# AppleHolic/pytorch_sound

Measured on AMD Instinct MI355X. Metric: audio-sec/s STFT+mel+fwd/bwd, higher is better.
Workload: dtype bf16; 1 GPU; configs[1]: Conv1d separator (4 x ResBlock1, C=256, on 513-bin magnitude), 22.05 kHz, STFT 1024/256, 80 mel, batch 32 x 2 s per GPU, Adam, bf16 autocast; global_batch=32, parallelism=dp1, model_params=5520386

## Files before the change

### pytorch_sound_amd/csrc/psnd_conv_chain.hip

```cpp
#include "psnd_conv_pair.h"

#include <atomic>
extern std::atomic<long long> g_conv_pair_stats[4];
std::atomic<long long> g_conv_chain_stats[2];

namespace {
using namespace pairk;

constexpr int CHAIN_MAX = 4;
struct ChainPair {
    const bf16_t *W1, *W2;
    const float *bias1, *bias2;
    bf16_t *mid_out, *out_raw, *out_act;
    int off1, dstep1, off2, dstep2;
    float act1_slope, act2_slope;
    const bf16_t *M1, *M2;
    float m1_slope, m2_slope;
};
struct ChainParams {
    const bf16_t *A, *res;
    long long R;
    int Lp, L, HP;
    int n_pairs, lo, ts;
    ChainPair d[CHAIN_MAX];
    long long *trace;
};
#define CHAIN_STAMP(i_)                                                                  \
    do {                                                                                 \
        if (p.trace && (threadIdx.x & 63) == 0) p.trace[((size_t)blockIdx.x * 8 + (threadIdx.x >> 6)) * 16 + (i_)] = __builtin_amdgcn_s_memtime(); \
    } while (0)

template <int C, int MR, bool BWD>
__global__ __launch_bounds__(512, 1) void conv_chain_kernel(ChainParams p) {
    constexpr int NT = 512, RU = RU8;
#ifndef PSND_CHAIN_AR
#define PSND_CHAIN_AR 3
#endif
    constexpr int AR = PSND_CHAIN_AR;
    static_assert(RU % AR == 0, "static ring slots");
    constexpr int RS = C + 8, PCS = C / 8, KSTEPS = C / 16, UNITS = 3 * KSTEPS;
    constexpr int MROWS = 32 * MR, MB = MR, BR = MROWS + 2 * HMAXP;
    static_assert(C == 256, "eight waves = eight column blocks of 32");
    static_assert(UNITS % RU == 0 && RU % 3 == 0, "the B ring turns whole");
    extern __shared__ __attribute__((aligned(16))) bf16_t smem[];
    __shared__ unsigned char s_in[MROWS];
    __shared__ __attribute__((aligned(16))) float s_bias[BWD ? 1 : 2][BWD ? 4 : 2 * C];
    __shared__ unsigned s_flag[2];
#ifndef PSND_CHAIN_FLAGS
#define PSND_CHAIN_FLAGS 0
#endif
    constexpr bool FLAGS = PSND_CHAIN_FLAGS != 0;
#ifndef PSND_CHAIN_EPRIO
#define PSND_CHAIN_EPRIO 2
#endif
    if (threadIdx.x < 2) s_flag[threadIdx.x] = 0;
    auto wait_flag = [&](int g, unsigned need) __attribute__((always_inline)) {
        if (!FLAGS || need == 0) return;
        volatile unsigned *f = &s_flag[g];
        int spins = 0;
        while (*f < need) {
            __builtin_amdgcn_s_sleep(1);
            if (++spins > (1 << 24)) __builtin_trap();
        }
        __builtin_amdgcn_fence(__ATOMIC_ACQUIRE, "workgroup");
    };
    auto signal_flag = [&]() __attribute__((always_inline)) {
        if (!FLAGS) return;
        __builtin_amdgcn_fence(__ATOMIC_RELEASE, "workgroup");
        if ((threadIdx.x & 63) == 0) __hip_atomic_fetch_add(&s_flag[threadIdx.x >> 8], 1u, __ATOMIC_RELAXED, __HIP_MEMORY_SCOPE_WORKGROUP);
    };
    bf16_t *sXa = smem, *sM = smem + BR * RS, *sXr = smem + 2 * BR * RS;
    const int tid = threadIdx.x, wave = tid >> 6, lane = tid & 63, li = lane & 31, kg = lane >> 5;
    const int cb = wave * 32 + 4 * kg, eo = li * RS + cb;
    const long long g0 = (long long)blockIdx.x * p.ts - p.lo;
    const unsigned t_bytes = (unsigned)((size_t)p.R * C * sizeof(bf16_t)), w_bytes = (unsigned)(3u * C * C * sizeof(bf16_t));
    const __amdgpu_buffer_rsrc_t rA = make_uniform_rsrc(p.A, (int)t_bytes), rR = make_uniform_rsrc(p.res, (int)t_bytes);
    CHAIN_STAMP(0);

    constexpr int NAU = (BR * PCS + NT - 1) / NT, NRU = MROWS * PCS / NT;
    static_assert(NRU * NT == MROWS * PCS, "raw tile tiling");
    uint4 ra[NAU], rr[BWD ? 1 : NRU];
#pragma unroll
    for (int u = 0; u < NAU; ++u) {
        const int idx = tid + NT * u, row = idx / PCS, pc = idx % PCS;
        const long long r = g0 - HMAXP + row;
        ra[u] = ld16(rA, (idx < BR * PCS && r >= 0 && r < p.R) ? (unsigned)(((size_t)r * C + 8 * pc) * sizeof(bf16_t)) : OOB);
    }
    if constexpr (!BWD) {
#pragma unroll
        for (int u = 0; u < NRU; ++u) {
            const int idx = tid + NT * u, row = idx / PCS, pc = idx % PCS;
            const long long r = g0 + row;
            rr[u] = ld16(rR, (r >= 0 && r < p.R) ? (unsigned)(((size_t)r * C + 8 * pc) * sizeof(bf16_t)) : OOB);
        }
    }
    unsigned char *sBits = reinterpret_cast<unsigned char *>(smem + 2 * BR * RS);
    constexpr int NMU = MROWS * PCS / NT;
    uint4 mq[BWD ? NMU : 1];
    auto mask_fetch = [&](const bf16_t *M) __attribute__((always_inline)) {
        const __amdgpu_buffer_rsrc_t rM = make_uniform_rsrc(M, (int)t_bytes);
#pragma unroll
        for (int u = 0; u < NMU; ++u) {
            const int idx = tid + NT * u, row = idx / PCS, pc = idx % PCS;
            const long long r = g0 + row;
            mq[u] = ld16(rM, (r >= 0 && r < p.R) ? (unsigned)(((size_t)r * C + 8 * pc) * sizeof(bf16_t)) : OOB);
        }
    };
    auto mask_commit = [&](int buf) __attribute__((always_inline)) {
#pragma unroll
        for (int u = 0; u < NMU; ++u) {
            const unsigned *w = reinterpret_cast<const unsigned *>(&mq[u]);
            unsigned byte = 0;
#pragma unroll
            for (int e = 0; e < 4; ++e) {
                byte |= ((int)(w[e] << 16) > 0 ? 1u : 0u) << (2 * e);
                byte |= ((int)w[e] > 0xffff ? 1u : 0u) << (2 * e + 1);
            }
            sBits[buf * (MROWS * PCS) + tid + NT * u] = (unsigned char)byte;
        }
    };
    if constexpr (BWD) mask_fetch(p.d[0].M1);
    uint4 rb[RU];
    const unsigned fwave = (unsigned)wave * (unsigned)KSTEPS * 1024u + (unsigned)lane * 16u;
    constexpr unsigned FTAP = (unsigned)(C / 32) * (unsigned)KSTEPS * 1024u;
    auto fetch_b = [&](auto slotc, __amdgpu_buffer_rsrc_t rW, int it) __attribute__((always_inline)) {
        constexpr int slot = decltype(slotc)::value, tap = slot % 3, ksl = slot / 3;
        const int ks = (RU / 3) * it + ksl;
        rb[slot] = __builtin_bit_cast(uint4, __builtin_amdgcn_raw_buffer_load_b128(rW, (int)(ks < KSTEPS ? fwave : OOB),
                                                                                    (int)((unsigned)tap * FTAP + (unsigned)ks * 1024u), 0));
    };
    {
        const __amdgpu_buffer_rsrc_t rW = make_uniform_rsrc(p.d[0].W1, (int)w_bytes);
        static_for<0, RU>([&](auto uc) __attribute__((always_inline)) { fetch_b(uc, rW, 0); });
    }
    ChainPair d = p.d[0];
    if constexpr (!BWD) {
        const float *bp = tid < C ? d.bias1 : d.bias2;
        s_bias[0][tid] = bp ? bp[tid & (C - 1)] : 0.f;
    }
    if (tid < MROWS) {
        const long long r = g0 + tid;
        const int l = (int)(((r % p.Lp) + p.Lp) % p.Lp);
        s_in[tid] = (r >= 0 && r < p.R && l >= p.HP && l < p.HP + p.L) ? 1 : 0;
    }
#pragma unroll
    for (int u = 0; u < NAU; ++u) {
        const int idx = tid + NT * u;
        if (idx < BR * PCS) *reinterpret_cast<uint4 *>(sXa + (idx / PCS) * RS + 8 * (idx % PCS)) = ra[u];
    }
    if constexpr (!BWD) {
#pragma unroll
        for (int u = 0; u < NRU; ++u) {
            const int idx = tid + NT * u;
            *reinterpret_cast<uint4 *>(sXr + (idx / PCS) * RS + 8 * (idx % PCS)) = rr[u];
        }
    } else {
        mask_commit(0);
    }
    for (int idx = tid; idx < 2 * HMAXP * PCS; idx += NT) {
        const int row = idx / PCS < HMAXP ? idx / PCS : MROWS + idx / PCS;
        *reinterpret_cast<uint4 *>(sM + row * RS + 8 * (idx % PCS)) = make_uint4(0, 0, 0, 0);
    }
    __syncthreads();
    CHAIN_STAMP(1);
    float xres[MB][16];
#pragma unroll
    for (int m = 0; m < MB; ++m)
#pragma unroll
        for (int g = 0; g < 4; ++g) {
            const bf16_t *src = BWD ? sXa + HMAXP * RS : sXr;
            const uint2 w = *reinterpret_cast<const uint2 *>(src + eo + m * 32 * RS + 8 * g);
            xres[m][4 * g] = __builtin_bit_cast(float, w.x << 16), xres[m][4 * g + 1] = __builtin_bit_cast(float, w.x & 0xffff0000u);
            xres[m][4 * g + 2] = __builtin_bit_cast(float, w.y << 16), xres[m][4 * g + 3] = __builtin_bit_cast(float, w.y & 0xffff0000u);
        }

    f32x16 acc[MB];
    auto zero_acc = [&]() __attribute__((always_inline)) {
#pragma unroll
        for (int m = 0; m < MB; ++m)
#pragma unroll
            for (int i = 0; i < 16; ++i) acc[m][i] = 0.f;
    };
    auto run_conv = [&](const bf16_t *src, int off0, int dstep, __amdgpu_buffer_rsrc_t rW, __amdgpu_buffer_rsrc_t rWn, unsigned need) __attribute__((always_inline)) {
        wait_flag(0, need);
        const bf16_t *ab[3];
#pragma unroll
        for (int t = 0; t < 3; ++t) ab[t] = src + (li + HMAXP + off0 + t * dstep) * RS + 8 * kg;
        auto afrag = [&](auto uc, int it, bf16x8 (&x)[MB]) __attribute__((always_inline)) {
            constexpr int u = decltype(uc)::value, tap = u % 3, ksl = u / 3;
            const bf16_t *pa = ab[tap] + 16 * ((RU / 3) * it + ksl);
#pragma unroll
            for (int m = 0; m < MB; ++m) x[m] = *reinterpret_cast<const bf16x8 *>(pa + m * 32 * RS);
        };
        bf16x8 xr[AR][MB];
        auto turns = [&](int it0, int it1) __attribute__((always_inline)) {
            static_for<0, AR - 1>([&](auto uc) __attribute__((always_inline)) { afrag(uc, it0, xr[decltype(uc)::value]); });
#pragma unroll 1
            for (int it = it0; it < it1; ++it) {
                static_for<0, RU>([&](auto uc) __attribute__((always_inline)) {
                    constexpr int u = decltype(uc)::value;
                    afrag(std::integral_constant<int, u + AR - 1>{}, it, xr[(u + AR - 1) % AR]);
                    const bf16x8 b = __builtin_bit_cast(bf16x8, rb[u]);
#pragma unroll
                    for (int m = 0; m < MB; ++m) acc[m] = __builtin_amdgcn_mfma_f32_32x32x16_bf16(b, xr[u % AR][m], acc[m], 0, 0, 0);
                    fetch_b(uc, it + 1 < UNITS / RU ? rW : rWn, it + 1 < UNITS / RU ? it + 1 : 0);
                    __builtin_amdgcn_sched_group_barrier(0x100, MB, 0);
                    __builtin_amdgcn_sched_group_barrier(0x008, MB, 0);
                    __builtin_amdgcn_sched_group_barrier(0x020, 1, 0);
                    __builtin_amdgcn_sched_barrier(0);
                });
            }
        };
        if constexpr (FLAGS) {
            turns(0, UNITS / RU / 2);
            wait_flag(1, need);
            turns(UNITS / RU / 2, UNITS / RU);
        } else {
            turns(0, UNITS / RU);
        }
    };
    auto copy_out = [&](const bf16_t *src, int row_off, bf16_t *dst) __attribute__((always_inline)) {
        if (wave >= 4) return;
        const __amdgpu_buffer_rsrc_t rO = make_uniform_rsrc(dst, (int)t_bytes);
        for (int idx = tid; idx < p.ts * PCS; idx += NT / 2) {
            const int i = p.lo + idx / PCS, pc = idx % PCS;
            const long long r = g0 + i;
            const uint4 v = *reinterpret_cast<const uint4 *>(src + (row_off + i) * RS + 8 * pc);
            __builtin_amdgcn_raw_buffer_store_b128(__builtin_bit_cast(__attribute__((ext_vector_type(4))) unsigned, v), rO,
                                                   (int)(r < p.R ? (unsigned)(((size_t)r * C + 8 * pc) * 2) : OOB), 0, 0);
        }
    };

    unsigned rmask[MB];
#pragma unroll
    for (int m = 0; m < MB; ++m) rmask[m] = s_in[m * 32 + li] ? 0xffffffffu : 0u;
    bf16_t *prev_raw = nullptr, *prev_act = nullptr;
    auto st8 = [&](bf16_t *row0, int m, int g, unsigned w0, unsigned w1) __attribute__((always_inline)) {
        *reinterpret_cast<uint2 *>(row0 + eo + m * 32 * RS + 8 * g) = make_uint2(w0, w1);
    };
    auto bias4 = [&](int buf, int conv, float4 (&bb)[4]) __attribute__((always_inline)) {
#pragma unroll
        for (int g = 0; g < 4; ++g) bb[g] = *reinterpret_cast<const float4 *>(&s_bias[buf][conv * C + cb + 8 * g]);
    };
    auto mask32 = [&](int buf, int m) __attribute__((always_inline)) {
        return *reinterpret_cast<const unsigned *>(sBits + buf * (MROWS * PCS) + (m * 32 + li) * PCS + 4 * wave) >> (4 * kg);
    };
    auto masked = [&](float v, float slope, unsigned bits, int j) __attribute__((always_inline)) {
        const unsigned sel = (unsigned)(((int)(bits << (31 - j))) >> 31);
        return __builtin_bit_cast(float, (__builtin_bit_cast(unsigned, v) & sel) | (__builtin_bit_cast(unsigned, v * slope) & ~sel));
    };
#pragma unroll 1
    for (int pp = 0; pp < p.n_pairs; ++pp) {
        const ChainPair dn = p.d[pp + 1 < p.n_pairs ? pp + 1 : pp];
        float bn = 0.f;
        if constexpr (!BWD) {
            const float *bp = tid < C ? dn.bias1 : dn.bias2;
            bn = bp ? bp[tid & (C - 1)] : 0.f;
        }
        const float sl1 = d.act1_slope, sl2 = d.act2_slope, ms1 = d.m1_slope, ms2 = d.m2_slope;
        const __amdgpu_buffer_rsrc_t rW1 = make_uniform_rsrc(d.W1, (int)w_bytes), rW2 = make_uniform_rsrc(d.W2, (int)w_bytes);
        const __amdgpu_buffer_rsrc_t rWn = make_uniform_rsrc(dn.W1, pp + 1 < p.n_pairs ? (int)w_bytes : 0);
        if constexpr (BWD) mask_fetch(d.M2);
        zero_acc();
        run_conv(sXa, d.off1, d.dstep1, rW1, rW2, 8u * pp);
        if constexpr (FLAGS) __builtin_amdgcn_s_setprio(PSND_CHAIN_EPRIO);
        CHAIN_STAMP(2 + 4 * pp);
        if (pp > 0) {
            if (prev_raw) copy_out(BWD ? sXa : sXr, BWD ? HMAXP : 0, prev_raw);
            if (!BWD && prev_act) copy_out(sXa, HMAXP, prev_act);
        }
        if constexpr (BWD) {
#pragma unroll
            for (int m = 0; m < MB; ++m) {
                const unsigned bits = mask32(0, m);
#pragma unroll
                for (int g = 0; g < 4; ++g) {
                    float v[4];
#pragma unroll
                    for (int j = 0; j < 4; ++j) v[j] = masked(acc[m][4 * g + j], ms1, bits, 8 * g + j);
                    st8(sM + HMAXP * RS, m, g, pack_bf16(v[0], v[1]) & rmask[m], pack_bf16(v[2], v[3]) & rmask[m]);
                }
            }
            mask_commit(1);
        } else {
            float4 bb[4];
            bias4(pp & 1, 0, bb);
#pragma unroll
            for (int m = 0; m < MB; ++m)
#pragma unroll
                for (int g = 0; g < 4; ++g) {
                    const float v0 = acc[m][4 * g] + bb[g].x, v1 = acc[m][4 * g + 1] + bb[g].y;
                    const float v2 = acc[m][4 * g + 2] + bb[g].z, v3 = acc[m][4 * g + 3] + bb[g].w;
                    st8(sM + HMAXP * RS, m, g, pack_bf16(fmaxf(v0, v0 * sl1), fmaxf(v1, v1 * sl1)) & rmask[m],
                        pack_bf16(fmaxf(v2, v2 * sl1), fmaxf(v3, v3 * sl1)) & rmask[m]);
                }
            s_bias[(pp + 1) & 1][tid] = bn;
        }
        if (pp == 1) CHAIN_STAMP(14);
        if constexpr (FLAGS) {
            signal_flag();
            __builtin_amdgcn_s_setprio(0);
        } else {
            __syncthreads();
        }
        CHAIN_STAMP(3 + 4 * pp);
        if constexpr (BWD) mask_fetch(dn.M1);
        zero_acc();
        run_conv(sM, d.off2, d.dstep2, rW2, rWn, 8u * pp + 4u);
        if constexpr (FLAGS) __builtin_amdgcn_s_setprio(PSND_CHAIN_EPRIO);
        CHAIN_STAMP(4 + 4 * pp);
        if (d.mid_out) copy_out(sM, HMAXP, d.mid_out);
        if constexpr (BWD) {
#pragma unroll
            for (int m = 0; m < MB; ++m) {
                const unsigned bits = mask32(1, m);
#pragma unroll
                for (int g = 0; g < 4; ++g) {
                    unsigned w[2];
#pragma unroll
                    for (int h = 0; h < 2; ++h) {
                        const int q = 4 * g + 2 * h;
                        const float v0 = masked(acc[m][q], ms2, bits, 8 * g + 2 * h) + xres[m][q];
                        const float v1 = masked(acc[m][q + 1], ms2, bits, 8 * g + 2 * h + 1) + xres[m][q + 1];
                        w[h] = pack_bf16(v0, v1) & rmask[m];
                        xres[m][q] = __builtin_bit_cast(float, w[h] << 16), xres[m][q + 1] = __builtin_bit_cast(float, w[h] & 0xffff0000u);
                    }
                    st8(sXa + HMAXP * RS, m, g, w[0], w[1]);
                }
            }
            mask_commit(0);
        } else {
            float4 bb[4];
            bias4(pp & 1, 1, bb);
#pragma unroll
            for (int m = 0; m < MB; ++m)
#pragma unroll
                for (int g = 0; g < 4; ++g) {
                    const float bq[4] = {bb[g].x, bb[g].y, bb[g].z, bb[g].w};
                    unsigned w[2], wa[2];
#pragma unroll
                    for (int h = 0; h < 2; ++h) {
                        const int q = 4 * g + 2 * h;
                        const float v0 = acc[m][q] + bq[2 * h] + xres[m][q], v1 = acc[m][q + 1] + bq[2 * h + 1] + xres[m][q + 1];
                        w[h] = pack_bf16(v0, v1) & rmask[m];
                        xres[m][q] = __builtin_bit_cast(float, w[h] << 16), xres[m][q + 1] = __builtin_bit_cast(float, w[h] & 0xffff0000u);
                        wa[h] = pack_bf16(fmaxf(v0, v0 * sl2), fmaxf(v1, v1 * sl2)) & rmask[m];
                    }
                    st8(sXr, m, g, w[0], w[1]);
                    st8(sXa + HMAXP * RS, m, g, wa[0], wa[1]);
                }
        }
        if (pp == 1) CHAIN_STAMP(15);
        if constexpr (FLAGS) {
            signal_flag();
            __builtin_amdgcn_s_setprio(0);
        } else {
            __syncthreads();
        }
        CHAIN_STAMP(5 + 4 * pp);
        prev_raw = d.out_raw, prev_act = d.out_act;
        d = dn;
    }
    if constexpr (FLAGS) __syncthreads();
    if (prev_raw) copy_out(BWD ? sXa : sXr, BWD ? HMAXP : 0, prev_raw);
    if (!BWD && prev_act) copy_out(sXa, HMAXP, prev_act);
}

int chain_loss(const int *taps, int n_pairs) {
    int loss = 0;
    for (int i = 0; i < n_pairs; ++i) loss += reach3(taps[4 * i], taps[4 * i + 1]) + reach3(taps[4 * i + 2], taps[4 * i + 3]);
    return loss - reach3(taps[0], taps[1]);
}
}

extern "C" int psnd_conv1d_cl_chain_rows(int C, int k, int n_pairs, const int *taps) {
    if (k != 3 || C != 256 || n_pairs < 1 || n_pairs > CHAIN_MAX || !taps) return 0;
    for (int i = 0; i < 2 * n_pairs; ++i)
        if (reach3(taps[2 * i], taps[2 * i + 1]) > HMAXP) return 0;
    const int ts = 64 - 2 * chain_loss(taps, n_pairs);
    return ts >= 16 ? ts : 0;
}

extern "C" int psnd_conv1d_cl_chain_plan(int C, int k, int n_pairs, const int *taps, int64_t R, int *mr_out) {
    const int ts2 = psnd_conv1d_cl_chain_rows(C, k, n_pairs, taps);
    if (!ts2) return 0;
    const int ts1 = ts2 - 32;
    (void)R;
    int mr = 2;
    if (const char *e = PSND_ENV("PSND_CHAIN_MR")) {
        const int f = atoi(e);
        if (f == 2 || (f == 1 && ts1 >= 8)) mr = f;
    }
    if (mr_out) *mr_out = mr;
    return mr == 1 ? ts1 : ts2;
}

extern "C" int psnd_conv1d_cl_chain(const void *A, const void *res, const psnd_chain_pair *pairs, int n_pairs, int64_t N, int Lp, int L, int HP,
                                    int C, int k, void *stream) {
    if (!A || !res || !pairs) PSND_FAIL(PSND_E_ARG, "conv1d_cl_chain: null pointer");
    const bool bwd = n_pairs >= 1 && pairs[0].M1 != nullptr;
    if (N < 0 || Lp <= 0 || L <= 0 || HP < 0 || Lp < L + HP) PSND_FAIL(PSND_E_SHAPE, "conv1d_cl_chain: N=%lld Lp=%d L=%d HP=%d", (long long)N, Lp, L, HP);
    if (n_pairs < 1 || n_pairs > CHAIN_MAX) PSND_FAIL(PSND_E_UNSUPPORTED, "conv1d_cl_chain: %d pairs (1 ... %d)", n_pairs, CHAIN_MAX);
    int taps[4 * CHAIN_MAX];
    for (int i = 0; i < n_pairs; ++i) {
        taps[4 * i] = pairs[i].off1, taps[4 * i + 1] = pairs[i].dstep1, taps[4 * i + 2] = pairs[i].off2, taps[4 * i + 3] = pairs[i].dstep2;
        if (!pairs[i].W1 || !pairs[i].W2) PSND_FAIL(PSND_E_ARG, "conv1d_cl_chain: pair %d without weights", i);
        if (bwd != (pairs[i].M1 != nullptr) || bwd != (pairs[i].M2 != nullptr))
            PSND_FAIL(PSND_E_ARG, "conv1d_cl_chain: pair %d: masks on every conv of the chain (the input-gradient form) or on none", i);
        if (bwd && (res != A || pairs[i].act1_slope != 1.f || pairs[i].act2_slope != 1.f || pairs[i].out_act || pairs[i].bias1 || pairs[i].bias2))
            PSND_FAIL(PSND_E_UNSUPPORTED, "conv1d_cl_chain: pair %d: the masked (input-gradient) form has res == A, no activation, no bias, no out_act", i);
        if (!(pairs[i].act1_slope >= 0.f && pairs[i].act1_slope <= 1.f && pairs[i].act2_slope >= 0.f && pairs[i].act2_slope <= 1.f))
            PSND_FAIL(PSND_E_UNSUPPORTED, "conv1d_cl_chain: activation slopes %g, %g of pair %d outside [0, 1]", pairs[i].act1_slope, pairs[i].act2_slope, i);
    }
    int mr = 2;
    const int ts = psnd_conv1d_cl_chain_plan(C, k, n_pairs, taps, N * (int64_t)Lp, &mr);
    if (!ts) PSND_FAIL(PSND_E_UNSUPPORTED, "conv1d_cl_chain: C=%d k=%d, %d pairs: only k = 3, C = 256, reach <= %d, >= 16 rows left of 64", C, k, n_pairs, HMAXP);
    if (N == 0) return PSND_OK;
    if ((size_t)N * Lp * C * 2 >= ((size_t)1 << 31)) PSND_FAIL(PSND_E_SHAPE, "conv1d_cl_chain: operand larger than 2 GB");
    ChainParams p;
    p.A = static_cast<const bf16_t *>(A), p.res = static_cast<const bf16_t *>(res);
    p.R = N * (int64_t)Lp, p.Lp = Lp, p.L = L, p.HP = HP;
    p.n_pairs = n_pairs, p.ts = ts, p.lo = (32 * mr - ts) / 2;
    for (int i = 0; i < CHAIN_MAX; ++i) {
        const psnd_chain_pair &s = pairs[i < n_pairs ? i : n_pairs - 1];
        ChainPair &d = p.d[i];
        d.W1 = static_cast<const bf16_t *>(s.W1), d.W2 = static_cast<const bf16_t *>(s.W2), d.bias1 = s.bias1, d.bias2 = s.bias2;
        d.mid_out = static_cast<bf16_t *>(s.mid_out), d.out_raw = static_cast<bf16_t *>(s.out_raw), d.out_act = static_cast<bf16_t *>(s.out_act);
        d.off1 = s.off1, d.dstep1 = s.dstep1, d.off2 = s.off2, d.dstep2 = s.dstep2, d.act1_slope = s.act1_slope, d.act2_slope = s.act2_slope;
        d.M1 = static_cast<const bf16_t *>(s.M1), d.M2 = static_cast<const bf16_t *>(s.M2), d.m1_slope = s.m1_slope, d.m2_slope = s.m2_slope;
    }
    p.trace = nullptr;
#ifdef PSND_TRACE
    {
        const char *tp = PSND_ENV("PSND_PAIR_TRACE_PTR");
        p.trace = tp ? reinterpret_cast<long long *>(strtoull(tp, nullptr, 0)) : nullptr;
    }
#endif
    const int64_t tiles = (p.R + ts - 1) / ts;
    constexpr int RS = 256 + 8;
    const int mrows = 32 * mr;
    const size_t lds = bwd ? (size_t)2 * (mrows + 2 * HMAXP) * RS * 2 + 2 * 256 * 8 : (size_t)(2 * (mrows + 2 * HMAXP) + mrows) * RS * 2;
    hipStream_t st = static_cast<hipStream_t>(stream);
    auto launch = [&](auto kern) {
        hipFuncSetAttribute(reinterpret_cast<const void *>(kern), hipFuncAttributeMaxDynamicSharedMemorySize, 128 * 1024);
        hipLaunchKernelGGL(kern, dim3((unsigned)tiles), dim3(512), lds, st, p);
    };
    if (bwd && mr == 2) launch(conv_chain_kernel<256, 2, true>);
    else if (bwd) launch(conv_chain_kernel<256, 1, true>);
    else if (mr == 2) launch(conv_chain_kernel<256, 2, false>);
    else launch(conv_chain_kernel<256, 1, false>);
    PSND_CHECK_LAUNCH("conv1d_cl_chain");
    g_conv_chain_stats[0]++;
    g_conv_chain_stats[1] += n_pairs;
    return PSND_OK;
}

extern "C" void psnd_conv_chain_stats(long long *out2) {
    out2[0] = g_conv_chain_stats[0].load(), out2[1] = g_conv_chain_stats[1].load();
}
```

Before: 107,700 audio-s/s.

## Micro-optimize conv chain kernel: packed epilogues, fused acc zeroing, batched copy-out

Several micro-optimizations land in the fused conv chain kernel. The accumulator zeroing is folded into the first MFMA turn, and epilogue math uses packed f32x2 ops with bfe/bfi inline asm for the masked leaky-ReLU backward. Mask bit packing switches to packed u16 inline asm. The prologue is reordered so bias loads and halo zeroing are issued earlier, with sched barriers between weight prefetches. Copy-out precomputes offsets, batches LDS reads before the stores, and uses all 512 threads for the final store. Together these aim to cut VALU and scheduling overhead, at the cost of more complex code and inline asm whose correctness must hold across edge cases.

```diff
diff --git a/pytorch_sound_amd/csrc/psnd_conv_chain.hip b/pytorch_sound_amd/csrc/psnd_conv_chain.hip
--- a/pytorch_sound_amd/csrc/psnd_conv_chain.hip
+++ b/pytorch_sound_amd/csrc/psnd_conv_chain.hip
@@ -77,6 +77,12 @@
     const __amdgpu_buffer_rsrc_t rA = make_uniform_rsrc(p.A, (int)t_bytes), rR = make_uniform_rsrc(p.res, (int)t_bytes);
     CHAIN_STAMP(0);
 
+    ChainPair d = p.d[0];
+    float b0 = 0.f;
+    if constexpr (!BWD) {
+        const float *bp = tid < C ? d.bias1 : d.bias2;
+        b0 = bp ? bp[tid & (C - 1)] : 0.f;
+    }
     constexpr int NAU = (BR * PCS + NT - 1) / NT, NRU = MROWS * PCS / NT;
     static_assert(NRU * NT == MROWS * PCS, "raw tile tiling");
     uint4 ra[NAU], rr[BWD ? 1 : NRU];
@@ -110,13 +116,15 @@
 #pragma unroll
         for (int u = 0; u < NMU; ++u) {
             const unsigned *w = reinterpret_cast<const unsigned *>(&mq[u]);
-            unsigned byte = 0;
+            unsigned s = 0;
 #pragma unroll
             for (int e = 0; e < 4; ++e) {
-                byte |= ((int)(w[e] << 16) > 0 ? 1u : 0u) << (2 * e);
-                byte |= ((int)w[e] > 0xffff ? 1u : 0u) << (2 * e + 1);
+                unsigned x;
+                asm("v_pk_sub_u16 %0, %1, %2" : "=v"(x) : "v"(w[e]), "v"(0x00010001u));
+                asm("v_pk_add_u16 %0, %1, %2 clamp" : "=v"(x) : "v"(x), "v"(0x00800080u));
+                s |= (x >> (15 - 2 * e)) & (0x00010001u << (2 * e));
             }
-            sBits[buf * (MROWS * PCS) + tid + NT * u] = (unsigned char)byte;
+            sBits[buf * (MROWS * PCS) + tid + NT * u] = (unsigned char)~(s | (s >> 15));
         }
     };
     if constexpr (BWD) mask_fetch(p.d[0].M1);
@@ -131,18 +139,21 @@
     };
     {
         const __amdgpu_buffer_rsrc_t rW = make_uniform_rsrc(p.d[0].W1, (int)w_bytes);
-        static_for<0, RU>([&](auto uc) __attribute__((always_inline)) { fetch_b(uc, rW, 0); });
-    }
-    ChainPair d = p.d[0];
-    if constexpr (!BWD) {
-        const float *bp = tid < C ? d.bias1 : d.bias2;
-        s_bias[0][tid] = bp ? bp[tid & (C - 1)] : 0.f;
+        static_for<0, RU>([&](auto uc) __attribute__((always_inline)) {
+            fetch_b(uc, rW, 0);
+            __builtin_amdgcn_sched_barrier(0);
+        });
     }
     if (tid < MROWS) {
         const long long r = g0 + tid;
         const int l = (int)(((r % p.Lp) + p.Lp) % p.Lp);
         s_in[tid] = (r >= 0 && r < p.R && l >= p.HP && l < p.HP + p.L) ? 1 : 0;
     }
+    for (int idx = tid; idx < 2 * HMAXP * PCS; idx += NT) {
+        const int row = idx / PCS < HMAXP ? idx / PCS : MROWS + idx / PCS;
+        *reinterpret_cast<uint4 *>(sM + row * RS + 8 * (idx % PCS)) = make_uint4(0, 0, 0, 0);
+    }
+    if constexpr (!BWD) s_bias[0][tid] = b0;
 #pragma unroll
     for (int u = 0; u < NAU; ++u) {
         const int idx = tid + NT * u;
@@ -157,30 +168,20 @@
     } else {
         mask_commit(0);
     }
-    for (int idx = tid; idx < 2 * HMAXP * PCS; idx += NT) {
-        const int row = idx / PCS < HMAXP ? idx / PCS : MROWS + idx / PCS;
-        *reinterpret_cast<uint4 *>(sM + row * RS + 8 * (idx % PCS)) = make_uint4(0, 0, 0, 0);
-    }
     __syncthreads();
     CHAIN_STAMP(1);
-    float xres[MB][16];
+    f32x2_t xres[MB][8];
 #pragma unroll
     for (int m = 0; m < MB; ++m)
 #pragma unroll
         for (int g = 0; g < 4; ++g) {
             const bf16_t *src = BWD ? sXa + HMAXP * RS : sXr;
             const uint2 w = *reinterpret_cast<const uint2 *>(src + eo + m * 32 * RS + 8 * g);
-            xres[m][4 * g] = __builtin_bit_cast(float, w.x << 16), xres[m][4 * g + 1] = __builtin_bit_cast(float, w.x & 0xffff0000u);
-            xres[m][4 * g + 2] = __builtin_bit_cast(float, w.y << 16), xres[m][4 * g + 3] = __builtin_bit_cast(float, w.y & 0xffff0000u);
+            xres[m][2 * g] = f32x2_t{__builtin_bit_cast(float, w.x << 16), __builtin_bit_cast(float, w.x & 0xffff0000u)};
+            xres[m][2 * g + 1] = f32x2_t{__builtin_bit_cast(float, w.y << 16), __builtin_bit_cast(float, w.y & 0xffff0000u)};
         }
 
     f32x16 acc[MB];
-    auto zero_acc = [&]() __attribute__((always_inline)) {
-#pragma unroll
-        for (int m = 0; m < MB; ++m)
-#pragma unroll
-            for (int i = 0; i < 16; ++i) acc[m][i] = 0.f;
-    };
     auto run_conv = [&](const bf16_t *src, int off0, int dstep, __amdgpu_buffer_rsrc_t rW, __amdgpu_buffer_rsrc_t rWn, unsigned need) __attribute__((always_inline)) {
         wait_flag(0, need);
         const bf16_t *ab[3];
@@ -193,41 +194,62 @@
             for (int m = 0; m < MB; ++m) x[m] = *reinterpret_cast<const bf16x8 *>(pa + m * 32 * RS);
         };
         bf16x8 xr[AR][MB];
-        auto turns = [&](int it0, int it1) __attribute__((always_inline)) {
+        auto turn = [&](int it, auto firstc) __attribute__((always_inline)) {
+            static_for<0, RU>([&](auto uc) __attribute__((always_inline)) {
+                constexpr int u = decltype(uc)::value;
+                afrag(std::integral_constant<int, u + AR - 1>{}, it, xr[(u + AR - 1) % AR]);
+                const bf16x8 b = __builtin_bit_cast(bf16x8, rb[u]);
+#pragma unroll
+                for (int m = 0; m < MB; ++m) {
+                    f32x16 c = acc[m];
+                    if constexpr (decltype(firstc)::value && u == 0) {
+#pragma unroll
+                        for (int i = 0; i < 16; ++i) c[i] = 0.f;
+                    }
+                    acc[m] = __builtin_amdgcn_mfma_f32_32x32x16_bf16(b, xr[u % AR][m], c, 0, 0, 0);
+                }
+                fetch_b(uc, it + 1 < UNITS / RU ? rW : rWn, it + 1 < UNITS / RU ? it + 1 : 0);
+                __builtin_amdgcn_sched_group_barrier(0x100, MB, 0);
+                __builtin_amdgcn_sched_group_barrier(0x008, MB, 0);
+                __builtin_amdgcn_sched_group_barrier(0x020, 1, 0);
+                __builtin_amdgcn_sched_barrier(0);
+            });
+        };
+        auto turns = [&](int it0, int it1, auto firstc) __attribute__((always_inline)) {
             static_for<0, AR - 1>([&](auto uc) __attribute__((always_inline)) { afrag(uc, it0, xr[decltype(uc)::value]); });
+            if constexpr (decltype(firstc)::value) turn(it0++, std::true_type{});
 #pragma unroll 1
-            for (int it = it0; it < it1; ++it) {
-                static_for<0, RU>([&](auto uc) __attribute__((always_inline)) {
-                    constexpr int u = decltype(uc)::value;
-                    afrag(std::integral_constant<int, u + AR - 1>{}, it, xr[(u + AR - 1) % AR]);
-                    const bf16x8 b = __builtin_bit_cast(bf16x8, rb[u]);
-#pragma unroll
-                    for (int m = 0; m < MB; ++m) acc[m] = __builtin_amdgcn_mfma_f32_32x32x16_bf16(b, xr[u % AR][m], acc[m], 0, 0, 0);
-                    fetch_b(uc, it + 1 < UNITS / RU ? rW : rWn, it + 1 < UNITS / RU ? it + 1 : 0);
-                    __builtin_amdgcn_sched_group_barrier(0x100, MB, 0);
-                    __builtin_amdgcn_sched_group_barrier(0x008, MB, 0);
-                    __builtin_amdgcn_sched_group_barrier(0x020, 1, 0);
-                    __builtin_amdgcn_sched_barrier(0);
-                });
-            }
+            for (int it = it0; it < it1; ++it) turn(it, std::false_type{});
         };
         if constexpr (FLAGS) {
-            turns(0, UNITS / RU / 2);
+            turns(0, UNITS / RU / 2, std::true_type{});
             wait_flag(1, need);
-            turns(UNITS / RU / 2, UNITS / RU);
+            turns(UNITS / RU / 2, UNITS / RU, std::false_type{});
         } else {
-            turns(0, UNITS / RU);
-        }
-    };
-    auto copy_out = [&](const bf16_t *src, int row_off, bf16_t *dst) __attribute__((always_inline)) {
-        if (wave >= 4) return;
+            turns(0, UNITS / RU, std::true_type{});
+        }
+    };
+    const int co_row = tid / PCS, co_pc = tid % PCS;
+    const long long co_left = p.R - (g0 + p.lo);
+    const int co_lim = co_left < (long long)p.ts ? (int)co_left : p.ts;
+    const unsigned co_goff = (unsigned)(((size_t)(g0 + p.lo + co_row) * C + 8 * co_pc) * sizeof(bf16_t));
+    auto copy_out = [&](const bf16_t *src, int row_off, bf16_t *dst, auto allc) __attribute__((always_inline)) {
+        constexpr bool ALL = decltype(allc)::value;
+        constexpr int NTH = ALL ? NT : NT / 2, RPR = NTH / PCS, NR = (MROWS + RPR - 1) / RPR, GR = 4;
+        if (!ALL && wave >= 4) return;
         const __amdgpu_buffer_rsrc_t rO = make_uniform_rsrc(dst, (int)t_bytes);
-        for (int idx = tid; idx < p.ts * PCS; idx += NT / 2) {
-            const int i = p.lo + idx / PCS, pc = idx % PCS;
-            const long long r = g0 + i;
-            const uint4 v = *reinterpret_cast<const uint4 *>(src + (row_off + i) * RS + 8 * pc);
-            __builtin_amdgcn_raw_buffer_store_b128(__builtin_bit_cast(__attribute__((ext_vector_type(4))) unsigned, v), rO,
-                                                   (int)(r < p.R ? (unsigned)(((size_t)r * C + 8 * pc) * 2) : OOB), 0, 0);
+        const bf16_t *s0 = src + (row_off + p.lo + co_row) * RS + 8 * co_pc;
+#pragma unroll
+        for (int r0 = 0; r0 < NR; r0 += GR) {
+            uint4 v[GR];
+#pragma unroll
+            for (int j = 0; j < GR; ++j)
+                if (r0 + j < NR && co_row + (r0 + j) * RPR < co_lim) v[j] = *reinterpret_cast<const uint4 *>(s0 + (r0 + j) * RPR * RS);
+#pragma unroll
+            for (int j = 0; j < GR; ++j)
+                if (r0 + j < NR && co_row + (r0 + j) * RPR < co_lim)
+                    __builtin_amdgcn_raw_buffer_store_b128(__builtin_bit_cast(__attribute__((ext_vector_type(4))) unsigned, v[j]), rO, (int)co_goff,
+                                                           (r0 + j) * RPR * C * (int)sizeof(bf16_t), 0);
         }
     };
 
@@ -245,9 +267,23 @@
     auto mask32 = [&](int buf, int m) __attribute__((always_inline)) {
         return *reinterpret_cast<const unsigned *>(sBits + buf * (MROWS * PCS) + (m * 32 + li) * PCS + 4 * wave) >> (4 * kg);
     };
-    auto masked = [&](float v, float slope, unsigned bits, int j) __attribute__((always_inline)) {
-        const unsigned sel = (unsigned)(((int)(bits << (31 - j))) >> 31);
-        return __builtin_bit_cast(float, (__builtin_bit_cast(unsigned, v) & sel) | (__builtin_bit_cast(unsigned, v * slope) & ~sel));
+    auto masked2 = [&](f32x2_t v, float slope, unsigned bits, int j) __attribute__((always_inline)) {
+        const f32x2_t s = v * slope;
+        unsigned sel0, sel1;
+        f32x2_t o;
+        asm("v_bfe_i32 %0, %1, %2, 1" : "=v"(sel0) : "v"(bits), "n"(j));
+        asm("v_bfe_i32 %0, %1, %2, 1" : "=v"(sel1) : "v"(bits), "n"(j + 1));
+        asm("v_bfi_b32 %0, %1, %2, %3" : "=v"(o.x) : "v"(sel0), "v"(v.x), "v"(s.x));
+        asm("v_bfi_b32 %0, %1, %2, %3" : "=v"(o.y) : "v"(sel1), "v"(v.y), "v"(s.y));
+        return o;
+    };
+    auto acc2 = [&](int m, int q) __attribute__((always_inline)) { return f32x2_t{acc[m][q], acc[m][q + 1]}; };
+    auto leaky2 = [&](f32x2_t v, float slope) __attribute__((always_inline)) {
+        const f32x2_t s = v * slope;
+        return pack_bf16(fmaxf(v.x, s.x), fmaxf(v.y, s.y));
+    };
+    auto unpack2 = [&](unsigned w) __attribute__((always_inline)) {
+        return f32x2_t{__builtin_bit_cast(float, w << 16), __builtin_bit_cast(float, w & 0xffff0000u)};
     };
 #pragma unroll 1
     for (int pp = 0; pp < p.n_pairs; ++pp) {
@@ -261,13 +297,12 @@
         const __amdgpu_buffer_rsrc_t rW1 = make_uniform_rsrc(d.W1, (int)w_bytes), rW2 = make_uniform_rsrc(d.W2, (int)w_bytes);
         const __amdgpu_buffer_rsrc_t rWn = make_uniform_rsrc(dn.W1, pp + 1 < p.n_pairs ? (int)w_bytes : 0);
         if constexpr (BWD) mask_fetch(d.M2);
-        zero_acc();
         run_conv(sXa, d.off1, d.dstep1, rW1, rW2, 8u * pp);
         if constexpr (FLAGS) __builtin_amdgcn_s_setprio(PSND_CHAIN_EPRIO);
         CHAIN_STAMP(2 + 4 * pp);
         if (pp > 0) {
-            if (prev_raw) copy_out(BWD ? sXa : sXr, BWD ? HMAXP : 0, prev_raw);
-            if (!BWD && prev_act) copy_out(sXa, HMAXP, prev_act);
+            if (prev_raw) copy_out(BWD ? sXa : sXr, BWD ? HMAXP : 0, prev_raw, std::false_type{});
+            if (!BWD && prev_act) copy_out(sXa, HMAXP, prev_act, std::false_type{});
         }
         if constexpr (BWD) {
 #pragma unroll
@@ -275,10 +310,8 @@
                 const unsigned bits = mask32(0, m);
 #pragma unroll
                 for (int g = 0; g < 4; ++g) {
-                    float v[4];
-#pragma unroll
-                    for (int j = 0; j < 4; ++j) v[j] = masked(acc[m][4 * g + j], ms1, bits, 8 * g + j);
-                    st8(sM + HMAXP * RS, m, g, pack_bf16(v[0], v[1]) & rmask[m], pack_bf16(v[2], v[3]) & rmask[m]);
+                    const f32x2_t v01 = masked2(acc2(m, 4 * g), ms1, bits, 8 * g), v23 = masked2(acc2(m, 4 * g + 2), ms1, bits, 8 * g + 2);
+                    st8(sM + HMAXP * RS, m, g, pack_bf16(v01.x, v01.y) & rmask[m], pack_bf16(v23.x, v23.y) & rmask[m]);
                 }
             }
             mask_commit(1);
@@ -289,10 +322,8 @@
             for (int m = 0; m < MB; ++m)
 #pragma unroll
                 for (int g = 0; g < 4; ++g) {
-                    const float v0 = acc[m][4 * g] + bb[g].x, v1 = acc[m][4 * g + 1] + bb[g].y;
-                    const float v2 = acc[m][4 * g + 2] + bb[g].z, v3 = acc[m][4 * g + 3] + bb[g].w;
-                    st8(sM + HMAXP * RS, m, g, pack_bf16(fmaxf(v0, v0 * sl1), fmaxf(v1, v1 * sl1)) & rmask[m],
-                        pack_bf16(fmaxf(v2, v2 * sl1), fmaxf(v3, v3 * sl1)) & rmask[m]);
+                    const f32x2_t v01 = acc2(m, 4 * g) + f32x2_t{bb[g].x, bb[g].y}, v23 = acc2(m, 4 * g + 2) + f32x2_t{bb[g].z, bb[g].w};
+                    st8(sM + HMAXP * RS, m, g, leaky2(v01, sl1) & rmask[m], leaky2(v23, sl1) & rmask[m]);
                 }
             s_bias[(pp + 1) & 1][tid] = bn;
         }
@@ -305,11 +336,10 @@
         }
         CHAIN_STAMP(3 + 4 * pp);
         if constexpr (BWD) mask_fetch(dn.M1);
-        zero_acc();
         run_conv(sM, d.off2, d.dstep2, rW2, rWn, 8u * pp + 4u);
         if constexpr (FLAGS) __builtin_amdgcn_s_setprio(PSND_CHAIN_EPRIO);
         CHAIN_STAMP(4 + 4 * pp);
-        if (d.mid_out) copy_out(sM, HMAXP, d.mid_out);
+        if (d.mid_out) copy_out(sM, HMAXP, d.mid_out, std::false_type{});
         if constexpr (BWD) {
 #pragma unroll
             for (int m = 0; m < MB; ++m) {
@@ -320,10 +350,9 @@
 #pragma unroll
                     for (int h = 0; h < 2; ++h) {
                         const int q = 4 * g + 2 * h;
-                        const float v0 = masked(acc[m][q], ms2, bits, 8 * g + 2 * h) + xres[m][q];
-                        const float v1 = masked(acc[m][q + 1], ms2, bits, 8 * g + 2 * h + 1) + xres[m][q + 1];
-                        w[h] = pack_bf16(v0, v1) & rmask[m];
-                        xres[m][q] = __builtin_bit_cast(float, w[h] << 16), xres[m][q + 1] = __builtin_bit_cast(float, w[h] & 0xffff0000u);
+                        const f32x2_t v = masked2(acc2(m, q), ms2, bits, 8 * g + 2 * h) + xres[m][q / 2];
+                        w[h] = pack_bf16(v.x, v.y) & rmask[m];
+                        xres[m][q / 2] = unpack2(w[h]);
                     }
                     st8(sXa + HMAXP * RS, m, g, w[0], w[1]);
                 }
@@ -336,15 +365,15 @@
             for (int m = 0; m < MB; ++m)
 #pragma unroll
                 for (int g = 0; g < 4; ++g) {
-                    const float bq[4] = {bb[g].x, bb[g].y, bb[g].z, bb[g].w};
+                    const f32x2_t bq[2] = {{bb[g].x, bb[g].y}, {bb[g].z, bb[g].w}};
                     unsigned w[2], wa[2];
 #pragma unroll
                     for (int h = 0; h < 2; ++h) {
                         const int q = 4 * g + 2 * h;
-                        const float v0 = acc[m][q] + bq[2 * h] + xres[m][q], v1 = acc[m][q + 1] + bq[2 * h + 1] + xres[m][q + 1];
-                        w[h] = pack_bf16(v0, v1) & rmask[m];
-                        xres[m][q] = __builtin_bit_cast(float, w[h] << 16), xres[m][q + 1] = __builtin_bit_cast(float, w[h] & 0xffff0000u);
-                        wa[h] = pack_bf16(fmaxf(v0, v0 * sl2), fmaxf(v1, v1 * sl2)) & rmask[m];
+                        const f32x2_t v = acc2(m, q) + bq[h] + xres[m][q / 2];
+                        w[h] = pack_bf16(v.x, v.y) & rmask[m];
+                        xres[m][q / 2] = unpack2(w[h]);
+                        wa[h] = leaky2(v, sl2) & rmask[m];
                     }
                     st8(sXr, m, g, w[0], w[1]);
                     st8(sXa + HMAXP * RS, m, g, wa[0], wa[1]);
@@ -362,8 +391,8 @@
         d = dn;
     }
     if constexpr (FLAGS) __syncthreads();
-    if (prev_raw) copy_out(BWD ? sXa : sXr, BWD ? HMAXP : 0, prev_raw);
-    if (!BWD && prev_act) copy_out(sXa, HMAXP, prev_act);
+    if (prev_raw) copy_out(BWD ? sXa : sXr, BWD ? HMAXP : 0, prev_raw, std::true_type{});
+    if (!BWD && prev_act) copy_out(sXa, HMAXP, prev_act, std::true_type{});
 }
 
 int chain_loss(const int *taps, int n_pairs) {
```

After: 109,100 audio-s/s, median of 6. 1.4% higher.
